# LuoweiZhou/VLP

Measured on NVIDIA H100. Metric: image_text_samples_per_sec, higher is better.
Workload: dtype bf16

## Files before the change

### vlp_b200/csrc/api.cu

```cuda
#include "../../include/vlpk.h"

#include <cstdlib>
#include <cstring>

#include "attn.cuh"
#include "decode.cuh"
#include "gemm.cuh"
#include "head.cuh"
#include "host.cuh"
#include "optim.cuh"
#include "rowops.cuh"
#include "tables.cuh"

using namespace vlpk;
typedef __nv_bfloat16 bf16;

namespace {

inline cudaStream_t S(void* s) { return reinterpret_cast<cudaStream_t>(s); }

enum { SITE_ATTN = 0, SITE_HID1 = 1, SITE_HID2 = 2 };
inline uint64_t site_of(uint64_t layer_id, int site) { return layer_id * 8 + site; }

inline DropoutCfg mk_drop(const VlpkDropout* d, float p, uint64_t site) {
// ... 322 lines not shown
  const long long i = (static_cast<long long>(blockIdx.x) * blockDim.x + threadIdx.x) * 8;
  if (i >= M * N) return;
  const long long r = i / N;
  const int c = static_cast<int>(i % N);
  const uint4 ud = *reinterpret_cast<const uint4*>(dy + r * lddy + c), uy = *reinterpret_cast<const uint4*>(y + r * ldy + c);
  const uint32_t wd[4] = {ud.x, ud.y, ud.z, ud.w}, wy[4] = {uy.x, uy.y, uy.z, uy.w};
  uint32_t o[4];
#pragma unroll
  for (int j = 0; j < 4; ++j) {
    const float2 d = unpack_bf16x2(wd[j]), v = unpack_bf16x2(wy[j]);
    o[j] = pack_bf16x2(v.x > 0.f ? d.x * scale : 0.f, v.y > 0.f ? d.y * scale : 0.f);
  }
  *reinterpret_cast<uint4*>(dpre + i) = make_uint4(o[0], o[1], o[2], o[3]);
}

int score_layer_fwd(const VlpkShape* s, int T, const AttnGroupKv* group, const VlpkLayerWeights* w, const void* x, const uint32_t* key_bits,
                    const uint32_t* query_bits, VlpkLayerActs* a, uint64_t layer_id, cudaStream_t st) {
  const int H = s->H, K = group != nullptr ? T - 1 : s->Lq, R = K + T;
  VLPK_TRY(qkv_fwd(s->B * R, H, w, x, a->qkv, st));
  const bf16* qkv = static_cast<const bf16*>(a->qkv);
  AttnGroupKv g;
  if (group != nullptr) {
    g = *group;
    g.text = qkv + H; g.ld_text = 3 * H; g.T = R; g.pos = 0;
  }
  AttnDesc ad;
  ad.B = s->B; ad.heads = s->heads; ad.Lkv = s->Lkv; ad.kv_slots = s->kv_slots;
  ad.q = qkv; ad.ld_q = 3 * H; ad.q_batch_stride = static_cast<int64_t>(R) * 3 * H;
  ad.k = qkv + H; ad.v = qkv + 2 * H; ad.kv_batch_stride = static_cast<int64_t>(R) * 3 * H;
  ad.ld_kv = group != nullptr ? 2 * H : 3 * H;
  ad.o = a->ctx; ad.ld_o = H; ad.o_batch_stride = static_cast<int64_t>(R) * H;
  ad.lse = a->lse;
  ad.drop = make_dropout(0.f, 0, 0);
  if (K > 0) {
    AttnDesc kd = ad;
    kd.Lq = K;
    kd.mask_bits = key_bits; kd.mask_rows = K;
    VLPK_TRY(launch_attn_fwd(kd, group != nullptr ? &g : nullptr, nullptr, st));
  }
  AttnDesc qd = ad;
  qd.Lq = T;
  qd.q = qkv + static_cast<size_t>(K) * 3 * H;
  qd.o = static_cast<bf16*>(a->ctx) + static_cast<size_t>(K) * H;
  qd.mask_bits = query_bits; qd.mask_rows = T;
  qd.lse = a->lse + static_cast<size_t>(s->B) * s->heads * K;
  AttnSelfKv sk;
  sk.k = qkv + static_cast<size_t>(K) * 3 * H + H;
  sk.v = qkv + static_cast<size_t>(K) * 3 * H + 2 * H;
  sk.ld = 3 * H; sk.batch_stride = static_cast<int64_t>(R) * 3 * H;
  VLPK_TRY(launch_attn_fwd(qd, group != nullptr ? &g : nullptr, &sk, st));
  VlpkShape rows = *s;
  rows.Lq = rows.Lkv = R;
  VLPK_TRY(attn_out_ln(&rows, w, x, a, 0.f, nullptr, layer_id, st));
  return ffn_fwd_impl(&rows, w, a, 0.f, nullptr, layer_id, st);
}

int score_stack_fwd(const VlpkShape* s, int T, int n_layers, const VlpkLayerWeights* w, const void* x, AttnGroupKv* group,
                    const void* const* prefix, const uint32_t* key_bits, const uint32_t* query_bits, VlpkLayerActs* acts, cudaStream_t st) {
  const void* cur = x;
  for (int i = 0; i < n_layers; ++i) {
    if (group != nullptr) group->prefix = prefix[i];
    VLPK_TRY(score_layer_fwd(s, T, group, &w[i], cur, key_bits, query_bits, &acts[i], i, st));
    cur = acts[i].y;
  }
  return 0;
}

size_t act_bytes(const VlpkShape* s, size_t rows, size_t kv_elems) {
  const size_t H = s->H, I = s->I, M = static_cast<size_t>(s->B) * rows;
  const size_t lse = (static_cast<size_t>(s->B) * s->heads * rows + 3) / 4 * 4;
  return 2 * (M * (3 * H + 5 * H + 2 * I) + kv_elems) + 4 * (lse + 4 * M);
}

}

#pragma GCC visibility push(default)
extern "C" {

int vlpk_version(void) { return VLPK_VERSION; }
int vlpk_debug_set_option(const char* name, int value) {
  VLPK_CHECK_ARG(name != nullptr, "set_option: null name");
  if (strcmp(name, "wgrad_stream") == 0) { g_wgrad_stream = value ? 1 : 0; return 0; }
  if (strcmp(name, "attn_tiled") == 0) { set_attn_tiled(value != 0); return 0; }
  set_error("set_option: unknown option '%s'", name);
  return -1;
}
int vlpk_debug_plan_gemm(int M, int N, int K, int a_mn, int b_mn, int nseg, int seg_rows, int epi, int bn, int splits, int* out2) {
  GemmDesc g;
  g.M = M; g.N = N; g.K = K;
  g.a_mn = a_mn != 0; g.b_mn = b_mn != 0;
  g.nseg = nseg; g.b_seg_rows = seg_rows;
  g.epi = epi; g.bn = bn; g.splits = splits;
  return plan_gemm(g, &out2[0], &out2[1]);
}
void vlpk_set_reserved_sms(int n) { set_reserved_sms(n); }
void vlpk_set_deterministic(int on) { set_deterministic(on != 0); }
const char* vlpk_last_error(void) { return get_error(); }

int vlpk_mask_pack(const void* mask, int dtype, int mode, int B, int rows, int kv, int64_t stride_b, int64_t stride_r, uint32_t* out,
                   void* stream) {
  VLPK_CHECK_ARG(mask != nullptr && out != nullptr, "mask_pack: null pointer");
  return launch_mask_pack(mask, dtype, mode, B, rows, kv, stride_b, stride_r, out, S(stream));
}

int vlpk_mask_synth(const int32_t* len_b, const int32_t* mode, int len_a, int B, int L, uint32_t* out, void* stream) {
  return launch_mask_synth(len_b, mode, len_a, B, L, out, S(stream));
}

int vlpk_mask_synth_grouped(const int32_t* len_b, int G, int len_a, int B, int T, uint32_t* out, void* stream) {
  return launch_mask_synth_grouped(len_b, G, len_a, B, T, out, S(stream));
}

int vlpk_linear_fwd(int M, int N, int K, const void* x, int64_t ldx, const void* w, int64_t ldw, const void* bias, void* y, int64_t ldy,
                    int act, const VlpkDropout* drop, uint64_t site, void* stream) {
  VLPK_CHECK_ARG(x && w && y, "linear_fwd: null pointer");
  VLPK_CHECK_ARG(act == VLPK_ACT_NONE || act == VLPK_ACT_RELU, "linear_fwd: act %d unsupported", act);
  const DropoutCfg dc = (act == VLPK_ACT_RELU && drop != nullptr) ? mk_drop(drop, drop->p, site) : make_dropout(0.f, 0, site);
  return fwd_linear(M, N, K, x, ldx, w, ldw, bias, y, ldy, act == VLPK_ACT_RELU ? EPI_RELU : EPI_STORE, nullptr, 0, dc, S(stream));
}

int vlpk_linear_bwd(int M, int N, int K, const void* x, int64_t ldx, const void* w, int64_t ldw, const void* y, int64_t ldy,
                    const void* dy, int64_t lddy, void* dpre, void* dx, int64_t lddx, float* dw, int64_t lddw, float* db, int act,
                    float p_drop, void* stream) {
  VLPK_CHECK_ARG(x && w && dy && dw, "linear_bwd: null pointer");
  cudaStream_t st = S(stream);
  const void* g = dy;
  int64_t ldg = lddy;
  if (act == VLPK_ACT_RELU) {
    VLPK_CHECK_ARG(y != nullptr && dpre != nullptr && N % 8 == 0, "linear_bwd: relu needs y, dpre and N %% 8 == 0");
    const long long n = static_cast<long long>(M) * N;
    LaunchScope scope(CAT_MISC, 6.0 * n, st);
    relu_bwd_kernel<<<static_cast<unsigned>((n / 8 + 255) / 256), 256, 0, st>>>(static_cast<bf16*>(dpre), static_cast<const bf16*>(dy),
                                                                             static_cast<const bf16*>(y), M, N, lddy, ldy,
                                                                             p_drop > 0.f ? 1.0f / (1.0f - p_drop) : 1.0f);
    VLPK_CUDA(cudaGetLastError());
    g = dpre;
    ldg = N;
  }
  if (db != nullptr) VLPK_TRY(launch_colsum(g, ldg, M, N, db, st));
  VLPK_TRY(wgrad_linear(M, N, K, g, ldg, x, ldx, dw, lddw, st));
  if (dx != nullptr) VLPK_TRY(dgrad_linear(M, N, K, g, ldg, w, ldw, dx, lddx, EPI_STORE, nullptr, 0, st));
  return 0;
}

static EmbedArgs mk_embed(int B, int L, int H, int R, int vis_input, const int64_t* ids, const int64_t* tt, const int64_t* pos,
                          const void* word_w, const void* pos_w, const void* type_w, const void* vis, const void* vpe,
                          const void* ln_g) {
  EmbedArgs a;
  a.B = B; a.L = L; a.H = H; a.R = R; a.vis_input = vis_input;
  a.ids = reinterpret_cast<const long long*>(ids);
  a.tt = reinterpret_cast<const long long*>(tt);
  a.pos = reinterpret_cast<const long long*>(pos);
  a.word = static_cast<const bf16*>(word_w); a.posw = static_cast<const bf16*>(pos_w); a.typew = static_cast<const bf16*>(type_w);
  a.vis = static_cast<const bf16*>(vis); a.vpe = static_cast<const bf16*>(vpe);
  a.gamma = static_cast<const bf16*>(ln_g);
  return a;
}

int vlpk_embed_fwd(int B, int L, int H, int R, int vis_input, const int64_t* ids, const int64_t* token_type, const int64_t* pos,
                   const void* word_w, const void* pos_w, const void* type_w, const void* vis, const void* vis_pe, const void* ln_g,
                   const void* ln_b, void* y, float* stats, const VlpkDropout* drop, uint64_t site, void* stream) {
  VLPK_CHECK_ARG(ids && word_w && pos_w && type_w && ln_g && ln_b && y, "embed_fwd: null pointer");
  EmbedArgs a = mk_embed(B, L, H, R, vis_input, ids, token_type, pos, word_w, pos_w, type_w, vis, vis_pe, ln_g);
  a.beta = static_cast<const bf16*>(ln_b);
  a.y = static_cast<bf16*>(y);
  a.stats = reinterpret_cast<float2*>(stats);
// ... 547 lines not shown
```

### vlp_b200/csrc/common.cuh

```cuda
#pragma once
#include <cuda.h>
#include <cuda_bf16.h>
#include <cuda_runtime.h>
#include <stdint.h>

#include "wgmma.cuh"

namespace vlpk {

__device__ __forceinline__ uint32_t smem_u32(const void* p) {
  return static_cast<uint32_t>(__cvta_generic_to_shared(p));
}

__device__ __forceinline__ uint32_t lane_id() { return threadIdx.x & 31u; }

__device__ __forceinline__ bool elect_one() {
  uint32_t pred = 0;
  asm volatile(
      "{\n\t"
      ".reg .pred P;\n\t"
      "elect.sync _|P, 0xffffffff;\n\t"
      "selp.u32 %0, 1, 0, P;\n\t"
      "}\n"
      : "=r"(pred));
  return pred != 0;
}

__device__ __forceinline__ void mbar_init(uint64_t* bar, uint32_t count) {
  asm volatile("mbarrier.init.shared::cta.b64 [%0], %1;" ::"r"(smem_u32(bar)), "r"(count) : "memory");
}
__device__ __forceinline__ void fence_mbar_init() {
  asm volatile("fence.mbarrier_init.release.cluster;" ::: "memory");
}
__device__ __forceinline__ void fence_proxy_async_smem() {
  asm volatile("fence.proxy.async.shared::cta;" ::: "memory");
}
__device__ __forceinline__ void mbar_arrive_expect_tx(uint64_t* bar, uint32_t bytes) {
  asm volatile("mbarrier.arrive.expect_tx.shared::cta.b64 _, [%0], %1;" ::"r"(smem_u32(bar)), "r"(bytes)
               : "memory");
}
__device__ __forceinline__ void mbar_arrive(uint64_t* bar) {
  asm volatile("mbarrier.arrive.shared::cta.b64 _, [%0];" ::"r"(smem_u32(bar)) : "memory");
}
__device__ __forceinline__ bool mbar_try_wait(uint64_t* bar, uint32_t parity) {
  uint32_t ok;
  asm volatile(
      "{\n\t"
      ".reg .pred P;\n\t"
      "mbarrier.try_wait.parity.shared::cta.b64 P, [%1], %2;\n\t"
      "selp.u32 %0, 1, 0, P;\n\t"
      "}\n"
      : "=r"(ok)
      : "r"(smem_u32(bar)), "r"(parity)
      : "memory");
  return ok != 0;
}
__device__ __forceinline__ void mbar_wait(uint64_t* bar, uint32_t parity) {
  uint32_t spins = 0;
  while (!mbar_try_wait(bar, parity)) {
    if (++spins > (1u << 28)) { __trap(); }
  }
}
__device__ __forceinline__ void mbar_wait_flag(uint64_t* bar, uint32_t parity, bool& timed_out) {
  uint32_t spins = 0;
  while (!timed_out && !mbar_try_wait(bar, parity)) {
    if (++spins > (1u << 28)) timed_out = true;
  }
}

__device__ __forceinline__ void pdl_launch_dependents() { asm volatile("griddepcontrol.launch_dependents;" ::: "memory"); }
__device__ __forceinline__ void pdl_wait() { asm volatile("griddepcontrol.wait;" ::: "memory"); }

__device__ __forceinline__ void tma_prefetch_desc(const CUtensorMap* m) {
  asm volatile("prefetch.tensormap [%0];" ::"l"(reinterpret_cast<uint64_t>(m)) : "memory");
}
__device__ __forceinline__ void tma_load_2d(void* dst, const CUtensorMap* m, uint64_t* bar, int c0, int c1) {
  asm volatile(
      "cp.async.bulk.tensor.2d.shared::cluster.global.tile.mbarrier::complete_tx::bytes [%0], [%1, {%3, %4}], [%2];"
      ::"r"(smem_u32(dst)), "l"(reinterpret_cast<uint64_t>(m)), "r"(smem_u32(bar)), "r"(c0), "r"(c1)
      : "memory");
}
__device__ __forceinline__ void tma_load_3d(void* dst, const CUtensorMap* m, uint64_t* bar, int c0, int c1,
                                            int c2) {
  asm volatile(
      "cp.async.bulk.tensor.3d.shared::cluster.global.tile.mbarrier::complete_tx::bytes [%0], [%1, {%3, %4, %5}], "
      "[%2];" ::"r"(smem_u32(dst)),
      "l"(reinterpret_cast<uint64_t>(m)), "r"(smem_u32(bar)), "r"(c0), "r"(c1), "r"(c2)
      : "memory");
}
__device__ __forceinline__ void tma_store_2d(const CUtensorMap* m, const void* src, int c0, int c1) {
  asm volatile("cp.async.bulk.tensor.2d.global.shared::cta.tile.bulk_group [%0, {%2, %3}], [%1];" ::"l"(
                   reinterpret_cast<uint64_t>(m)),
               "r"(smem_u32(src)), "r"(c0), "r"(c1)
               : "memory");
}
__device__ __forceinline__ void tma_store_3d(const CUtensorMap* m, const void* src, int c0, int c1, int c2) {
  asm volatile("cp.async.bulk.tensor.3d.global.shared::cta.tile.bulk_group [%0, {%2, %3, %4}], [%1];" ::"l"(
                   reinterpret_cast<uint64_t>(m)),
               "r"(smem_u32(src)), "r"(c0), "r"(c1), "r"(c2)
               : "memory");
}
__device__ __forceinline__ void tma_reduce_add_2d(const CUtensorMap* m, const void* src, int c0, int c1) {
  asm volatile("cp.reduce.async.bulk.tensor.2d.global.shared::cta.add.tile.bulk_group [%0, {%2, %3}], [%1];" ::"l"(
                   reinterpret_cast<uint64_t>(m)),
               "r"(smem_u32(src)), "r"(c0), "r"(c1)
               : "memory");
}
__device__ __forceinline__ void tma_reduce_add_3d(const CUtensorMap* m, const void* src, int c0, int c1, int c2) {
  asm volatile("cp.reduce.async.bulk.tensor.3d.global.shared::cta.add.tile.bulk_group [%0, {%2, %3, %4}], [%1];" ::"l"(
                   reinterpret_cast<uint64_t>(m)),
               "r"(smem_u32(src)), "r"(c0), "r"(c1), "r"(c2)
               : "memory");
}
__device__ __forceinline__ void tma_store_commit() { asm volatile("cp.async.bulk.commit_group;" ::: "memory"); }
template <int N>
__device__ __forceinline__ void tma_store_wait_read() {
  asm volatile("cp.async.bulk.wait_group.read %0;" ::"n"(N) : "memory");
}
template <int N>
__device__ __forceinline__ void tma_store_wait() {
  asm volatile("cp.async.bulk.wait_group %0;" ::"n"(N) : "memory");
}

__device__ __forceinline__ void wgmma_fence() { asm volatile("wgmma.fence.sync.aligned;" ::: "memory"); }
__device__ __forceinline__ void wgmma_commit() { asm volatile("wgmma.commit_group.sync.aligned;" ::: "memory"); }
template <int N>
__device__ __forceinline__ void wgmma_wait() {
  asm volatile("wgmma.wait_group.sync.aligned %0;" ::"n"(N) : "memory");
}
template <uint32_t N>
__device__ __forceinline__ void setmaxnreg_dec() { asm volatile("setmaxnreg.dec.sync.aligned.u32 %0;" ::"n"(N)); }
template <uint32_t N>
__device__ __forceinline__ void setmaxnreg_inc() { asm volatile("setmaxnreg.inc.sync.aligned.u32 %0;" ::"n"(N)); }
template <int N>
__device__ __forceinline__ void reg_fence(float (&d)[N]) {
#pragma unroll
  for (int i = 0; i < N; ++i) asm volatile("" : "+f"(d[i])::"memory");
}

__device__ __forceinline__ uint64_t wgmma_desc_sw128(uint32_t saddr, uint32_t lbo_bytes, uint32_t sbo_bytes) {
  uint64_t d = 0;
  d |= static_cast<uint64_t>((saddr & 0x3FFFFu) >> 4);
  d |= static_cast<uint64_t>((lbo_bytes >> 4) & 0x3FFFu) << 16;
  d |= static_cast<uint64_t>((sbo_bytes >> 4) & 0x3FFFu) << 32;
  d |= 1ull << 62;
  return d;
}

__device__ __forceinline__ uint32_t pack_bf16x2(float lo, float hi) {
  __nv_bfloat162 v = __floats2bfloat162_rn(lo, hi);
  return *reinterpret_cast<uint32_t*>(&v);
}
__device__ __forceinline__ float2 unpack_bf16x2(uint32_t u) {
  __nv_bfloat162 v = *reinterpret_cast<__nv_bfloat162*>(&u);
  return __bfloat1622float2(v);
}
__device__ __forceinline__ float bf16_round(float x) { return __bfloat162float(__float2bfloat16_rn(x)); }

__device__ __forceinline__ float fast_ex2(float x) {
  float y;
  asm("ex2.approx.ftz.f32 %0, %1;" : "=f"(y) : "f"(x));
  return y;
// ... 81 lines not shown
```

### vlp_b200/csrc/gemm.cu

```cuda
#include "gemm.cuh"

#include <cstdlib>

#include "host.cuh"
#include "rowops.cuh"

namespace vlpk {

static constexpr int BM = 128;
static constexpr int BK = 64;
static constexpr int NUM_THREADS = 384;
static constexpr int PRODUCER_REGS = 24;
static constexpr int CONSUMER_REGS = 240;
static constexpr int STG_BYTES = 64 * 128;
static constexpr int STG_PER_CONSUMER = 4;
static constexpr int SMEM_MAX = 232448;
static constexpr int BN = 128;

struct GemmTmaps {
  CUtensorMap a;
  CUtensorMap b[3];
  CUtensorMap d0;
  CUtensorMap d1;
  CUtensorMap aux;
};

struct GemmArgs {
  int M, N, K;
  int b_seg_rows;
  int splits;
  int split_slices;
  const __nv_bfloat16* bias[3];
  float relu_scale;
  DropoutCfg drop;
  float* colsum;
};

template <int STAGES>
struct SmemLayout {
  static constexpr int A_BYTES = BM * BK * 2;
  static constexpr int B_BYTES = BN * BK * 2;
  static constexpr int STAGE_BYTES = A_BYTES + B_BYTES;
  static constexpr int OFF_STG = STAGES * STAGE_BYTES;
  static constexpr int OFF_BAR = OFF_STG + 2 * STG_PER_CONSUMER * STG_BYTES;
  static constexpr int NUM_BARS = 3 * STAGES + 2;
  static constexpr int TOTAL = OFF_BAR + NUM_BARS * 8;
  static constexpr int DYN_BYTES = TOTAL + 1024;
  static_assert(DYN_BYTES <= SMEM_MAX, "shared memory budget exceeded");
};

struct StageCount {
  static constexpr int value = (SMEM_MAX - 1024 - 2 * STG_PER_CONSUMER * STG_BYTES - 256) / (BM * BK * 2 + BN * BK * 2);
};

__device__ __forceinline__ void wg_bar_sync(int cw) {
  asm volatile("bar.sync %0, 128;" ::"r"(cw + 1) : "memory");
}

template <bool A_MN, bool B_MN, int EPI>
__global__ void __launch_bounds__(NUM_THREADS, 1)
gemm_kernel(const __grid_constant__ GemmTmaps tm, const GemmArgs args) {
  constexpr int STAGES = StageCount::value;
  using L = SmemLayout<STAGES>;
  extern __shared__ uint8_t smem_raw[];
  uint8_t* smem = reinterpret_cast<uint8_t*>((reinterpret_cast<uintptr_t>(smem_raw) + 1023) & ~uintptr_t(1023));

  uint64_t* bars = reinterpret_cast<uint64_t*>(smem + L::OFF_BAR);
  uint64_t* full_bar = bars;
  uint64_t* empty_bar = bars + 2 * STAGES;
  uint64_t* aux_bar = bars + 3 * STAGES;
  constexpr bool HAS_AUX = (EPI == EPI_ADD || EPI == EPI_MUL || EPI == EPI_DRELU);

  pdl_launch_dependents();
  const int wg = __shfl_sync(0xffffffffu, threadIdx.x >> 7, 0);
  const int lane = threadIdx.x & 31;

  const int num_m = (args.M + BM - 1) / BM;
  const int num_n = (args.N + BN - 1) / BN;
  const int total_kb = (args.K + BK - 1) / BK;
  const int kb_per = (total_kb + args.splits - 1) / args.splits;
  const int num_work = num_m * num_n * args.splits;

  if (threadIdx.x == 0) {
    tma_prefetch_desc(&tm.a);
    tma_prefetch_desc(&tm.b[0]);
    tma_prefetch_desc(&tm.d0);
    if (HAS_AUX) tma_prefetch_desc(&tm.aux);
    for (int i = 0; i < 2 * STAGES; ++i) mbar_init(&full_bar[i], 1);
    for (int i = 0; i < STAGES; ++i) mbar_init(&empty_bar[i], 4);
    for (int i = 0; i < 2; ++i) mbar_init(&aux_bar[i], 1);
    fence_mbar_init();
  }
  __syncthreads();
  pdl_wait();

  if (wg == 0) {
    setmaxnreg_dec<PRODUCER_REGS>();
    if (threadIdx.x < 32) {
      int stage = 0;
      uint32_t phase = 0;
      int item = 0;
      for (int w = blockIdx.x; w < num_work; w += gridDim.x, ++item) {
        uint64_t* fb = full_bar + (item & 1) * STAGES;
        const int n_blk = w % num_n;
        const int m_blk = (w / num_n) % num_m;
        const int split = w / (num_n * num_m);
        const int kb0 = split * kb_per;
        const int kb1 = min(total_kb, kb0 + kb_per);
        const int m0 = m_blk * BM;
        for (int kb = kb0; kb < kb1; ++kb) {
          mbar_wait(&empty_bar[stage], phase ^ 1u);
          if (elect_one()) {
            uint8_t* sA = smem + stage * L::STAGE_BYTES;
            uint8_t* sB = sA + L::A_BYTES;
            mbar_arrive_expect_tx(&fb[stage], L::STAGE_BYTES);
            if (!A_MN) {
              tma_load_2d(sA, &tm.a, &fb[stage], kb * BK, m0);
            } else {
#pragma unroll
              for (int j = 0; j < BM / 64; ++j) tma_load_2d(sA + j * 8192, &tm.a, &fb[stage], m0 + j * 64, kb * BK);
            }
            if (!B_MN) {
              const int n0 = n_blk * BN;
              const int seg = n0 / args.b_seg_rows;
              tma_load_2d(sB, &tm.b[seg], &fb[stage], kb * BK, n0 - seg * args.b_seg_rows);
            } else {
              const int k0 = kb * BK;
              const int seg = k0 / args.b_seg_rows;
#pragma unroll
              for (int j = 0; j < BN / 64; ++j)
                tma_load_2d(sB + j * 8192, &tm.b[seg], &fb[stage], n_blk * BN + j * 64, k0 - seg * args.b_seg_rows);
            }
          }
          __syncwarp();
          if (++stage == STAGES) {
            stage = 0;
            phase ^= 1u;
          }
        }
      }
    }
  } else {
    setmaxnreg_inc<CONSUMER_REGS>();
    const int cw = wg - 1;
    const int t = threadIdx.x - 128 * wg;
    const int fr = (t >> 5) * 16 + (lane >> 2);
    const int fc = (lane & 3) * 2;
    const bool store_thread = (t == 0);
    const uint64_t dseed = drop_seed(args.drop);
    constexpr bool HAS_BIAS = !B_MN && (EPI == EPI_STORE || EPI == EPI_GELU || EPI == EPI_RELU);
    uint8_t* stg_base = smem + L::OFF_STG + cw * STG_PER_CONSUMER * STG_BYTES;
    const uint32_t a_base = smem_u32(smem);
    const uint32_t b_base = smem_u32(smem) + L::A_BYTES;
    uint64_t* fb = full_bar + cw * STAGES;
    int stage = 0;
    uint32_t phases = 0;
    uint32_t box_seq = 0;
    uint32_t aux_phase = 0;
    bool timed_out = false;
    float acc[2][BN / 2];
#pragma unroll
    for (int i = 0; i < BN / 2; ++i) acc[0][i] = acc[1][i] = 0.f;
    for (int w = blockIdx.x + cw * gridDim.x; w < num_work; w += 2 * gridDim.x) {
      const int w_other = w - static_cast<int>(gridDim.x);
      if (w_other >= static_cast<int>(blockIdx.x)) {
        const int split_o = w_other / (num_n * num_m);
        const int kb0_o = split_o * kb_per;
        stage = (stage + min(total_kb, kb0_o + kb_per) - kb0_o) % STAGES;
      }
      const int n_blk = w % num_n;
      const int m_blk = (w / num_n) % num_m;
      const int split = w / (num_n * num_m);
      const int kb0 = split * kb_per;
      const int kb1 = min(total_kb, kb0 + kb_per);
      const int n0 = n_blk * BN;

      int prev_stage = 0;
      for (int kb = kb0; kb < kb1; ++kb) {
        mbar_wait_flag(&fb[stage], (phases >> stage) & 1u, timed_out);
        phases ^= 1u << stage;
        const uint32_t sa = a_base + stage * L::STAGE_BYTES;
        const uint32_t sb = b_base + stage * L::STAGE_BYTES;
        reg_fence(acc[0]);
        reg_fence(acc[1]);
        wgmma_fence();
#pragma unroll
        for (int k = 0; k < BK / 16; ++k) {
          const uint64_t bdesc = B_MN ? wgmma_desc_sw128(sb + k * 2048, 8192, 1024) : wgmma_desc_sw128(sb + k * 32, 16, 1024);
#pragma unroll
          for (int h = 0; h < 2; ++h) {
            const uint32_t sah = sa + h * 8192;
            const uint64_t adesc = A_MN ? wgmma_desc_sw128(sah + k * 2048, 8192, 1024) : wgmma_desc_sw128(sah + k * 32, 16, 1024);
            wgmma_m64n128k16_ss<A_MN ? 1 : 0, B_MN ? 1 : 0>(acc[h], adesc, bdesc, (kb > kb0 || k > 0) ? 1u : 0u);
          }
        }
        wgmma_commit();
        if (HAS_AUX && kb == kb0) {
          static_assert(STG_PER_CONSUMER == 2 * (BN / 64), "one staging box per aux box of a tile");
          wg_bar_sync(cw);
          if (store_thread) {
            tma_store_wait_read<0>();
            fence_proxy_async_smem();
            mbar_arrive_expect_tx(&aux_bar[cw], STG_PER_CONSUMER * STG_BYTES);
#pragma unroll
            for (int b = 0; b < STG_PER_CONSUMER; ++b)
              tma_load_2d(stg_base + b * STG_BYTES, &tm.aux, &aux_bar[cw], n0 + (b & 1) * 64, m_blk * BM + (b >> 1) * 64);
          }
        }
        wgmma_wait<1>();
        reg_fence(acc[0]);
        reg_fence(acc[1]);
        if (kb > kb0 && lane == 0) mbar_arrive(&empty_bar[prev_stage]);
        prev_stage = stage;
        if (++stage == STAGES) stage = 0;
      }
      wgmma_wait<0>();
      reg_fence(acc[0]);
      reg_fence(acc[1]);
      if (lane == 0) mbar_arrive(&empty_bar[prev_stage]);

      if (EPI == EPI_REDUCE_F32) {
        constexpr int NBOX = BN / 32;
#pragma unroll
        for (int h = 0; h < 2; ++h) {
          const int m0 = m_blk * BM + h * 64;
#pragma unroll
          for (int c = 0; c < NBOX; ++c) {
            uint8_t* stg = stg_base + (box_seq % STG_PER_CONSUMER) * STG_BYTES;
            if (store_thread) tma_store_wait_read<STG_PER_CONSUMER - 1>();
            wg_bar_sync(cw);
#pragma unroll
            for (int j = 0; j < 8; ++j) {
              const int i = c * 16 + 2 * j;
              const int r = fr + 8 * (j & 1), col = 8 * (j >> 1) + fc;
              *reinterpret_cast<float2*>(stg + r * 128 + (((col >> 2) ^ (r & 7)) << 4) + (col & 3) * 4) = make_float2(acc[h][i], acc[h][i + 1]);
            }
            fence_proxy_async_smem();
            wg_bar_sync(cw);
            if (store_thread) {
              tma_reduce_add_3d(&tm.d0, stg, n0 + c * 32, m0, args.split_slices ? split : 0);
              tma_store_commit();
            }
            ++box_seq;
          }
        }
      } else {
        constexpr int NBOX = BN / 64;
        if (HAS_AUX) {
          mbar_wait_flag(&aux_bar[cw], aux_phase, timed_out);
          aux_phase ^= 1u;
        }
        const __nv_bfloat16* bp = nullptr;
        int bias_off = 0;
        if (HAS_BIAS) {
          const int seg = n0 / args.b_seg_rows;
          bp = args.bias[seg];
          bias_off = seg * args.b_seg_rows;
        }
#pragma unroll
        for (int h = 0; h < 2; ++h) {
          const int m0 = m_blk * BM + h * 64;
          int nh = n0;
          const __nv_bfloat16* bph = bp;
          uint64_t dsh = dseed;
          asm volatile("" : "+r"(nh), "+l"(bph), "+l"(dsh));
#pragma unroll
          for (int c = 0; c < NBOX; ++c) {
            uint8_t* stg = (EPI == EPI_GELU) ? stg_base + (box_seq & 1u) * 2 * STG_BYTES : stg_base + (box_seq % STG_PER_CONSUMER) * STG_BYTES;
            uint8_t* stg_g = stg + STG_BYTES;
            if (store_thread) {
              if (EPI == EPI_GELU) tma_store_wait_read<STG_PER_CONSUMER / 2 - 1>(); else tma_store_wait_read<STG_PER_CONSUMER - 1>();
            }
            wg_bar_sync(cw);
#pragma unroll
            for (int j = 0; j < 16; ++j) {
              const int i = c * 32 + 2 * j;
              const int r = fr + 8 * (j & 1), col = 8 * (j >> 1) + fc;
              const int n = nh + c * 64 + col;
              const long long m = m0 + r;
              const int so = r * 128 + (((col >> 3) ^ (r & 7)) << 4) + (col & 7) * 2;
              float v0 = acc[h][i], v1 = acc[h][i + 1];
              if (HAS_BIAS) {
                if (bph != nullptr && n < args.N) {
                  const float2 bb = unpack_bf16x2(__ldg(reinterpret_cast<const unsigned int*>(bph + n - bias_off)));
                  v0 += bb.x;
                  v1 += bb.y;
                }
              }
              if (EPI == EPI_GELU) {
                float g0, d0, g1, d1;
                gelu_and_grad(v0, g0, d0);
                gelu_and_grad(v1, g1, d1);
                *reinterpret_cast<uint32_t*>(stg + so) = pack_bf16x2(d0, d1);
                *reinterpret_cast<uint32_t*>(stg_g + so) = pack_bf16x2(g0, g1);
                continue;
              }
              if (EPI == EPI_RELU) {
                uint32_t keep = 0xFFu;
                if (args.drop.p > 0.f)
                  keep = dropout_keep8(dsh, args.drop.site, (static_cast<uint64_t>(m) * args.N + (n - fc)) >> 3, args.drop.thresh16);
                v0 = fmaxf(v0, 0.f);
                v1 = fmaxf(v1, 0.f);
                v0 = ((keep >> fc) & 1u) ? v0 * args.drop.scale : 0.f;
                v1 = ((keep >> (fc + 1)) & 1u) ? v1 * args.drop.scale : 0.f;
              } else if (EPI == EPI_ADD || EPI == EPI_MUL || EPI == EPI_DRELU) {
                const float2 x = unpack_bf16x2(*reinterpret_cast<const uint32_t*>(stg + so));
                if (EPI == EPI_ADD) {
                  v0 += x.x;
                  v1 += x.y;
                } else if (EPI == EPI_MUL) {
                  v0 *= x.x;
                  v1 *= x.y;
                } else {
                  v0 = x.x > 0.f ? v0 * args.relu_scale : 0.f;
                  v1 = x.y > 0.f ? v1 * args.relu_scale : 0.f;
                }
              }
              *reinterpret_cast<uint32_t*>(stg + so) = pack_bf16x2(v0, v1);
            }
            fence_proxy_async_smem();
            wg_bar_sync(cw);
            if (store_thread) {
              tma_store_2d(&tm.d0, stg, nh + c * 64, m0);
              if (EPI == EPI_GELU) tma_store_2d(&tm.d1, stg_g, nh + c * 64, m0);
              tma_store_commit();
            }
            if (EPI != EPI_GELU && args.colsum != nullptr) {
              const int col = t & 63, r0 = (t >> 6) * 32;
              float acc_c = 0.f;
#pragma unroll 8
              for (int rr = r0; rr < r0 + 32; ++rr) {
                const __nv_bfloat16 v = *reinterpret_cast<const __nv_bfloat16*>(stg + rr * 128 + (((col >> 3) ^ (rr & 7)) << 4) + (col & 7) * 2);
                acc_c += __bfloat162float(v);
              }
              if (nh + c * 64 + col < args.N) atomicAdd(args.colsum + nh + c * 64 + col, acc_c);
            }
            ++box_seq;
          }
        }
      }
    }
    if (store_thread) tma_store_wait<0>();
    if (timed_out) __trap();
  }
}

template <bool A_MN, bool B_MN, int EPI>
static int launch_inst(const GemmTmaps& tm, const GemmArgs& args, int num_work, cudaStream_t stream) {
  constexpr int STAGES = StageCount::value;
  using L = SmemLayout<STAGES>;
  auto kfn = gemm_kernel<A_MN, B_MN, EPI>;
  static bool attr_set = false;
  if (!attr_set) {
    VLPK_CUDA(cudaFuncSetAttribute(kfn, cudaFuncAttributeMaxDynamicSharedMemorySize, L::DYN_BYTES));
    attr_set = true;
  }
  const int max_ctas = gemm_sms();
  const int ctas = num_work < max_ctas ? num_work : max_ctas;
  LaunchScope scope(A_MN ? CAT_GEMM_WGRAD : (B_MN ? CAT_GEMM_DGRAD : CAT_GEMM_FWD), 2.0 * args.M * args.N * args.K, stream);
  VLPK_CUDA(launch_ex(kfn, dim3(ctas), dim3(NUM_THREADS), L::DYN_BYTES, stream, 1, tm, args));
  return 0;
}

static int dispatch(const GemmDesc& g, const GemmTmaps& tm, const GemmArgs& args, int num_work, cudaStream_t s) {
  if (!g.a_mn && !g.b_mn) {
    switch (g.epi) {
      case EPI_STORE: return launch_inst<false, false, EPI_STORE>(tm, args, num_work, s);
      case EPI_GELU: return launch_inst<false, false, EPI_GELU>(tm, args, num_work, s);
      case EPI_RELU: return launch_inst<false, false, EPI_RELU>(tm, args, num_work, s);
      default: break;
    }
  } else if (!g.a_mn && g.b_mn) {
    switch (g.epi) {
      case EPI_STORE: return launch_inst<false, true, EPI_STORE>(tm, args, num_work, s);
      case EPI_ADD: return launch_inst<false, true, EPI_ADD>(tm, args, num_work, s);
      case EPI_MUL: return launch_inst<false, true, EPI_MUL>(tm, args, num_work, s);
      case EPI_DRELU: return launch_inst<false, true, EPI_DRELU>(tm, args, num_work, s);
      case EPI_REDUCE_F32: return launch_inst<false, true, EPI_REDUCE_F32>(tm, args, num_work, s);
      default: break;
    }
  } else if (g.a_mn && g.b_mn) {
    if (g.epi == EPI_REDUCE_F32) return launch_inst<true, true, EPI_REDUCE_F32>(tm, args, num_work, s);
    if (g.epi == EPI_STORE) return launch_inst<true, true, EPI_STORE>(tm, args, num_work, s);
  }
  set_error("gemm: unsupported (a_mn=%d, b_mn=%d, epi=%d) combination", (int)g.a_mn, (int)g.b_mn, g.epi);
  return -1;
}

static double tile_cost(int M, int N, int total_kb, int splits, bool reduce) {
  const int num_m = (M + BM - 1) / BM;
  const int num_n = (N + BN - 1) / BN;
  const long long tiles = static_cast<long long>(num_m) * num_n * splits;
  const int slots = deterministic() ? num_sms() : gemm_sms();
  const long long rounds = (tiles + slots - 1) / slots;
  const int kb_per = (total_kb + splits - 1) / splits;
  const double mainloop = kb_per * (128.0 + double(BN));
  const double epi = (reduce ? 3.0 : 1.5) * BN;
  return rounds * (mainloop + epi + 60.0);
}

int plan_gemm(const GemmDesc& g, int* bn_out, int* splits_out) {
  const int seg_rows = g.nseg > 1 ? g.b_seg_rows : (g.b_mn ? g.K : g.N);
  const int total_kb = (g.K + BK - 1) / BK;
  const bool reduce = (g.epi == EPI_REDUCE_F32);
  VLPK_CHECK_ARG(g.bn == 0 || g.bn == BN, "gemm: no valid tile configuration (bn=%d; tiles are %d wide)", g.bn, BN);
  VLPK_CHECK_ARG(g.nseg == 1 || seg_rows % (g.b_mn ? BK : BN) == 0, "gemm: segment rows %d not tile aligned", seg_rows);
  int splits = 1;
  if (reduce) {
    const int max_s = total_kb / 8 > 0 ? total_kb / 8 : 1;
    if (g.splits > 0) {
      splits = g.splits < max_s ? g.splits : max_s;
    } else {
      double best = 1e300;
      for (int s = 1; s <= max_s; ++s) {
        const double c = tile_cost(g.M, g.N, total_kb, s, reduce);
        if (c < best) {
          best = c;
          splits = s;
        }
      }
    }
  }
  if (splits > total_kb) splits = total_kb;
  {
    const int kb_per = (total_kb + splits - 1) / splits;
    splits = (total_kb + kb_per - 1) / kb_per;
  }
  *bn_out = BN;
  *splits_out = splits;
  return 0;
}

int launch_gemm(const GemmDesc& g, cudaStream_t stream) {
  VLPK_CHECK_ARG(g.M > 0 && g.N > 0 && g.K > 0, "gemm: empty problem M=%d N=%d K=%d", g.M, g.N, g.K);
  VLPK_CHECK_ARG(g.N % 8 == 0, "gemm: N=%d must be a multiple of 8", g.N);
  VLPK_CHECK_ARG(g.nseg >= 1 && g.nseg <= 3, "gemm: nseg=%d", g.nseg);
  const int seg_rows = g.nseg > 1 ? g.b_seg_rows : (g.b_mn ? g.K : g.N);
  const bool reduce = (g.epi == EPI_REDUCE_F32);
  VLPK_CHECK_ARG(g.splits <= 1 || reduce, "gemm: split-K needs EPI_REDUCE_F32");
  VLPK_CHECK_ARG(g.b_rows == 0 || (g.nseg == 1 && g.b_rows <= (g.b_mn ? g.K : g.N)), "gemm: b_rows=%d needs a single B segment", g.b_rows);

  int bn = BN, splits = 1;
  VLPK_TRY(plan_gemm(g, &bn, &splits));

  GemmTmaps tm;
  memset(&tm, 0, sizeof(tm));
  if (!g.a_mn) {
    VLPK_TRY(make_tmap_2d(&tm.a, TM_BF16, g.A, g.K, g.M, g.lda, BK, BM));
  } else {
    VLPK_TRY(make_tmap_2d(&tm.a, TM_BF16, g.A, g.M, g.K, g.lda, 64, BK));
  }
  for (int s = 0; s < g.nseg; ++s) {
    if (!g.b_mn) {
      const int rows = g.nseg > 1 ? seg_rows : (g.b_rows > 0 ? g.b_rows : g.N);
      VLPK_TRY(make_tmap_2d(&tm.b[s], TM_BF16, g.B[s], g.K, rows, g.ldb, BK, bn));
    } else {
      const int rows = g.nseg > 1 ? seg_rows : (g.b_rows > 0 ? g.b_rows : g.K);
      VLPK_TRY(make_tmap_2d(&tm.b[s], TM_BF16, g.B[s], g.N, rows, g.ldb, 64, BK));
    }
  }
  for (int s = g.nseg; s < 3; ++s) tm.b[s] = tm.b[0];
  if (reduce) {
    VLPK_CHECK_ARG(g.split_stride == 0 || (g.split_stride % 4 == 0 && g.split_stride >= static_cast<int64_t>(g.M) * g.ldd0),
                   "gemm: split_stride %lld must be a multiple of 4 and cover M x ldd0", (long long)g.split_stride);
    const uint64_t dims[3] = {static_cast<uint64_t>(g.N), static_cast<uint64_t>(g.M), static_cast<uint64_t>(g.split_stride ? splits : 1)};
    const uint64_t strides[2] = {static_cast<uint64_t>(g.ldd0) * 4,
                                 static_cast<uint64_t>(g.split_stride ? g.split_stride : static_cast<int64_t>(g.M) * g.ldd0) * 4};
    const uint32_t box[3] = {32, 64, 1};
    VLPK_TRY(make_tmap(&tm.d0, TM_F32, 3, g.D0, dims, strides, box));
    tm.d1 = tm.d0;
  } else {
    VLPK_TRY(make_tmap_2d(&tm.d0, TM_BF16, g.D0, g.N, g.M, g.ldd0, 64, 64));
    if (g.epi == EPI_GELU) {
      VLPK_CHECK_ARG(g.D1 != nullptr, "gemm: EPI_GELU needs D1");
      VLPK_TRY(make_tmap_2d(&tm.d1, TM_BF16, g.D1, g.N, g.M, g.ldd1, 64, 64));
    } else {
      tm.d1 = tm.d0;
    }
  }
  VLPK_CHECK_ARG(g.colsum == nullptr || (!reduce && g.epi != EPI_GELU), "gemm: colsum fusion is for single-output bf16 epilogues");
  if (g.epi == EPI_ADD || g.epi == EPI_MUL || g.epi == EPI_DRELU) {
    VLPK_CHECK_ARG(g.aux != nullptr && (g.ld_aux % 8) == 0 && (reinterpret_cast<uintptr_t>(g.aux) & 15u) == 0,
                   "gemm: aux must be 16-byte aligned with ld %% 8 == 0");
    VLPK_TRY(make_tmap_2d(&tm.aux, TM_BF16, g.aux, g.N, g.M, g.ld_aux, 64, 64));
  } else {
    tm.aux = tm.d0;
  }

  GemmArgs a;
  a.M = g.M;
  a.N = g.N;
  a.K = g.K;
  a.b_seg_rows = seg_rows;
  a.splits = splits;
  a.split_slices = (reduce && g.split_stride > 0) ? 1 : 0;
  for (int s = 0; s < 3; ++s) a.bias[s] = (s < g.nseg) ? g.bias[s] : nullptr;
  a.relu_scale = g.relu_scale;
  a.colsum = g.colsum;
  a.drop = g.drop;

  const int num_m = (g.M + BM - 1) / BM;
  const int num_n = (g.N + bn - 1) / bn;
  const int num_work = num_m * num_n * splits;
  return dispatch(g, tm, a, num_work, stream);
}

int launch_gemm_split_slices(GemmDesc g, int slot, cudaStream_t stream) {
  VLPK_CHECK_ARG(g.epi == EPI_REDUCE_F32 && g.split_stride == 0, "gemm: split slices are for EPI_REDUCE_F32 into one D0");
  int bn = 0, splits = 1;
  VLPK_TRY(plan_gemm(g, &bn, &splits));
  if (splits == 1) return launch_gemm(g, stream);
  VLPK_CHECK_ARG(g.ldd0 == g.N, "gemm: split slices need a dense D0 (ldd0 %lld != N %d)", (long long)g.ldd0, g.N);
  const long long n = static_cast<long long>(g.M) * g.N;
  float* part = scratch_f32(slot, static_cast<size_t>(n) * splits, stream);
  if (part == nullptr) return -1;
  VLPK_CUDA(cudaMemsetAsync(part, 0, static_cast<size_t>(n) * splits * sizeof(float), stream));
  float* out = static_cast<float*>(g.D0);
  g.D0 = part;
  g.splits = splits;
  g.split_stride = n;
  VLPK_TRY(launch_gemm(g, stream));
  return launch_sum_parts(part, splits, n, out, stream);
}

}
```

### vlp_b200/csrc/gemm.cuh

```cuda
#pragma once
#include "common.cuh"

namespace vlpk {

enum Epi : int {
  EPI_STORE = 0,
  EPI_GELU = 1,
  EPI_RELU = 2,
  EPI_ADD = 3,
  EPI_MUL = 4,
  EPI_DRELU = 5,
  EPI_REDUCE_F32 = 6,
};

struct GemmDesc {
  int M = 0, N = 0, K = 0;
  bool a_mn = false;
  const void* A = nullptr;
  int64_t lda = 0;
  bool b_mn = false;
  int nseg = 1;
  const void* B[3] = {nullptr, nullptr, nullptr};
  int64_t ldb = 0;
  int b_seg_rows = 0;
  int b_rows = 0;
  const __nv_bfloat16* bias[3] = {nullptr, nullptr, nullptr};
  void* D0 = nullptr;
  int64_t ldd0 = 0;
  void* D1 = nullptr;
  int64_t ldd1 = 0;
  const __nv_bfloat16* aux = nullptr;
  int64_t ld_aux = 0;
  int epi = EPI_STORE;
  float relu_scale = 1.0f;
  DropoutCfg drop = {0.f, 1.f, 0u, 0ull, 0ull, nullptr};
  float* colsum = nullptr;
  int splits = 1;
  int64_t split_stride = 0;
  int bn = 0;
};

int launch_gemm(const GemmDesc& g, cudaStream_t stream);
int plan_gemm(const GemmDesc& g, int* bn_out, int* splits_out);
int launch_gemm_split_slices(GemmDesc g, int slot, cudaStream_t stream);

}
```

Baseline: 5342.

## Multicast B tiles across 2-CTA clusters in the persistent GEMM kernel

Launches the persistent warp-specialized GEMM as 2-CTA clusters along M. Each CTA loads one 64-column half of the shared B tile and multicasts it via TMA to both CTAs, which halves B global/L2 traffic. Empty barriers now count arrivals from both CTAs, and cluster syncs are added at start and end. The cost is cross-CTA coupling that can stall a pair, odd-M padding waste, and occupancy limited by the cluster count.

```diff
diff --git a/vlp_b200/csrc/api.cu b/vlp_b200/csrc/api.cu
--- a/vlp_b200/csrc/api.cu
+++ b/vlp_b200/csrc/api.cu
@@ -428,6 +428,7 @@
   VLPK_CHECK_ARG(name != nullptr, "set_option: null name");
   if (strcmp(name, "wgrad_stream") == 0) { g_wgrad_stream = value ? 1 : 0; return 0; }
   if (strcmp(name, "attn_tiled") == 0) { set_attn_tiled(value != 0); return 0; }
+  if (strcmp(name, "gemm_cluster") == 0) { set_gemm_cluster(value != 0); return 0; }
   set_error("set_option: unknown option '%s'", name);
   return -1;
 }
diff --git a/vlp_b200/csrc/common.cuh b/vlp_b200/csrc/common.cuh
--- a/vlp_b200/csrc/common.cuh
+++ b/vlp_b200/csrc/common.cuh
@@ -42,6 +42,15 @@
 __device__ __forceinline__ void mbar_arrive(uint64_t* bar) {
   asm volatile("mbarrier.arrive.shared::cta.b64 _, [%0];" ::"r"(smem_u32(bar)) : "memory");
 }
+__device__ __forceinline__ void mbar_arrive_cluster(uint64_t* bar, uint32_t cta) {
+  asm volatile(
+      "{\n\t"
+      ".reg .b32 ra;\n\t"
+      "mapa.shared::cluster.u32 ra, %0, %1;\n\t"
+      "mbarrier.arrive.release.cluster.shared::cluster.b64 _, [ra];\n\t"
+      "}\n" ::"r"(smem_u32(bar)), "r"(cta)
+      : "memory");
+}
 __device__ __forceinline__ bool mbar_try_wait(uint64_t* bar, uint32_t parity) {
   uint32_t ok;
   asm volatile(
@@ -71,6 +80,15 @@
 __device__ __forceinline__ void pdl_launch_dependents() { asm volatile("griddepcontrol.launch_dependents;" ::: "memory"); }
 __device__ __forceinline__ void pdl_wait() { asm volatile("griddepcontrol.wait;" ::: "memory"); }
 
+__device__ __forceinline__ uint32_t cluster_ctarank() {
+  uint32_t r;
+  asm volatile("mov.u32 %0, %%cluster_ctarank;" : "=r"(r));
+  return r;
+}
+__device__ __forceinline__ void cluster_sync() {
+  asm volatile("barrier.cluster.arrive.release;\n\tbarrier.cluster.wait.acquire;" ::: "memory");
+}
+
 __device__ __forceinline__ void tma_prefetch_desc(const CUtensorMap* m) {
   asm volatile("prefetch.tensormap [%0];" ::"l"(reinterpret_cast<uint64_t>(m)) : "memory");
 }
@@ -78,6 +96,13 @@
   asm volatile(
       "cp.async.bulk.tensor.2d.shared::cluster.global.tile.mbarrier::complete_tx::bytes [%0], [%1, {%3, %4}], [%2];"
       ::"r"(smem_u32(dst)), "l"(reinterpret_cast<uint64_t>(m)), "r"(smem_u32(bar)), "r"(c0), "r"(c1)
+      : "memory");
+}
+__device__ __forceinline__ void tma_load_2d_multicast(void* dst, const CUtensorMap* m, uint64_t* bar, int c0, int c1, uint16_t cta_mask) {
+  asm volatile(
+      "cp.async.bulk.tensor.2d.shared::cluster.global.tile.mbarrier::complete_tx::bytes.multicast::cluster [%0], [%1, {%3, %4}], [%2], "
+      "%5;" ::"r"(smem_u32(dst)),
+      "l"(reinterpret_cast<uint64_t>(m)), "r"(smem_u32(bar)), "r"(c0), "r"(c1), "h"(cta_mask)
       : "memory");
 }
 __device__ __forceinline__ void tma_load_3d(void* dst, const CUtensorMap* m, uint64_t* bar, int c0, int c1,
diff --git a/vlp_b200/csrc/gemm.cu b/vlp_b200/csrc/gemm.cu
--- a/vlp_b200/csrc/gemm.cu
+++ b/vlp_b200/csrc/gemm.cu
@@ -30,6 +30,8 @@
   int b_seg_rows;
   int splits;
   int split_slices;
+  int cluster;
+  int num_mp;
   const __nv_bfloat16* bias[3];
   float relu_scale;
   DropoutCfg drop;
@@ -53,6 +55,8 @@
   static constexpr int value = (SMEM_MAX - 1024 - 2 * STG_PER_CONSUMER * STG_BYTES - 256) / (BM * BK * 2 + BN * BK * 2);
 };
 
+__device__ __forceinline__ int cluster_rank(int csize) { return csize > 1 ? static_cast<int>(cluster_ctarank()) : 0; }
+
 __device__ __forceinline__ void wg_bar_sync(int cw) {
   asm volatile("bar.sync %0, 128;" ::"r"(cw + 1) : "memory");
 }
@@ -75,11 +79,14 @@
   const int wg = __shfl_sync(0xffffffffu, threadIdx.x >> 7, 0);
   const int lane = threadIdx.x & 31;
 
-  const int num_m = (args.M + BM - 1) / BM;
+  const int csize = args.cluster;
+  const int cid = blockIdx.x >> (csize - 1);
+  const int num_clusters = gridDim.x >> (csize - 1);
+  const int num_mp = args.num_mp;
   const int num_n = (args.N + BN - 1) / BN;
   const int total_kb = (args.K + BK - 1) / BK;
   const int kb_per = (total_kb + args.splits - 1) / args.splits;
-  const int num_work = num_m * num_n * args.splits;
+  const int num_work = num_mp * num_n * args.splits;
 
   if (threadIdx.x == 0) {
     tma_prefetch_desc(&tm.a);
@@ -87,11 +94,11 @@
     tma_prefetch_desc(&tm.d0);
     if (HAS_AUX) tma_prefetch_desc(&tm.aux);
     for (int i = 0; i < 2 * STAGES; ++i) mbar_init(&full_bar[i], 1);
-    for (int i = 0; i < STAGES; ++i) mbar_init(&empty_bar[i], 4);
+    for (int i = 0; i < STAGES; ++i) mbar_init(&empty_bar[i], 4 * csize);
     for (int i = 0; i < 2; ++i) mbar_init(&aux_bar[i], 1);
     fence_mbar_init();
   }
-  __syncthreads();
+  if (csize > 1) cluster_sync(); else __syncthreads();
   pdl_wait();
 
   if (wg == 0) {
@@ -100,11 +107,11 @@
       int stage = 0;
       uint32_t phase = 0;
       int item = 0;
-      for (int w = blockIdx.x; w < num_work; w += gridDim.x, ++item) {
+      for (int w = cid; w < num_work; w += num_clusters, ++item) {
         uint64_t* fb = full_bar + (item & 1) * STAGES;
         const int n_blk = w % num_n;
-        const int m_blk = (w / num_n) % num_m;
-        const int split = w / (num_n * num_m);
+        const int m_blk = (w / num_n) % num_mp * csize + cluster_rank(csize);
+        const int split = w / (num_n * num_mp);
         const int kb0 = split * kb_per;
         const int kb1 = min(total_kb, kb0 + kb_per);
         const int m0 = m_blk * BM;
@@ -120,16 +127,23 @@
 #pragma unroll
               for (int j = 0; j < BM / 64; ++j) tma_load_2d(sA + j * 8192, &tm.a, &fb[stage], m0 + j * 64, kb * BK);
             }
-            if (!B_MN) {
-              const int n0 = n_blk * BN;
-              const int seg = n0 / args.b_seg_rows;
-              tma_load_2d(sB, &tm.b[seg], &fb[stage], kb * BK, n0 - seg * args.b_seg_rows);
-            } else {
-              const int k0 = kb * BK;
-              const int seg = k0 / args.b_seg_rows;
-#pragma unroll
-              for (int j = 0; j < BN / 64; ++j)
-                tma_load_2d(sB + j * 8192, &tm.b[seg], &fb[stage], n_blk * BN + j * 64, k0 - seg * args.b_seg_rows);
+            const int j0 = csize > 1 ? cluster_ctarank() : 0;
+            const int j1 = csize > 1 ? j0 + 1 : BN / 64;
+            for (int j = j0; j < j1; ++j) {
+              int c0, c1, seg;
+              if (!B_MN) {
+                const int n0 = n_blk * BN;
+                seg = n0 / args.b_seg_rows;
+                c0 = kb * BK;
+                c1 = n0 - seg * args.b_seg_rows + j * 64;
+              } else {
+                const int k0 = kb * BK;
+                seg = k0 / args.b_seg_rows;
+                c0 = n_blk * BN + j * 64;
+                c1 = k0 - seg * args.b_seg_rows;
+              }
+              if (csize > 1) tma_load_2d_multicast(sB + j * 8192, &tm.b[seg], &fb[stage], c0, c1, 0x3);
+              else tma_load_2d(sB + j * 8192, &tm.b[seg], &fb[stage], c0, c1);
             }
           }
           __syncwarp();
@@ -161,16 +175,20 @@
     float acc[2][BN / 2];
 #pragma unroll
     for (int i = 0; i < BN / 2; ++i) acc[0][i] = acc[1][i] = 0.f;
-    for (int w = blockIdx.x + cw * gridDim.x; w < num_work; w += 2 * gridDim.x) {
-      const int w_other = w - static_cast<int>(gridDim.x);
-      if (w_other >= static_cast<int>(blockIdx.x)) {
-        const int split_o = w_other / (num_n * num_m);
+    auto release = [&](int s) {
+      mbar_arrive(&empty_bar[s]);
+      if (csize > 1) mbar_arrive_cluster(&empty_bar[s], cluster_ctarank() ^ 1u);
+    };
+    for (int w = cid + cw * num_clusters; w < num_work; w += 2 * num_clusters) {
+      const int w_other = w - num_clusters;
+      if (w_other >= cid) {
+        const int split_o = w_other / (num_n * num_mp);
         const int kb0_o = split_o * kb_per;
         stage = (stage + min(total_kb, kb0_o + kb_per) - kb0_o) % STAGES;
       }
       const int n_blk = w % num_n;
-      const int m_blk = (w / num_n) % num_m;
-      const int split = w / (num_n * num_m);
+      const int m_blk = (w / num_n) % num_mp * csize + cluster_rank(csize);
+      const int split = w / (num_n * num_mp);
       const int kb0 = split * kb_per;
       const int kb1 = min(total_kb, kb0 + kb_per);
       const int n0 = n_blk * BN;
@@ -210,14 +228,14 @@
         wgmma_wait<1>();
         reg_fence(acc[0]);
         reg_fence(acc[1]);
-        if (kb > kb0 && lane == 0) mbar_arrive(&empty_bar[prev_stage]);
+        if (kb > kb0 && lane == 0) release(prev_stage);
         prev_stage = stage;
         if (++stage == STAGES) stage = 0;
       }
       wgmma_wait<0>();
       reg_fence(acc[0]);
       reg_fence(acc[1]);
-      if (lane == 0) mbar_arrive(&empty_bar[prev_stage]);
+      if (lane == 0) release(prev_stage);
 
       if (EPI == EPI_REDUCE_F32) {
         constexpr int NBOX = BN / 32;
@@ -343,45 +361,68 @@
     if (store_thread) tma_store_wait<0>();
     if (timed_out) __trap();
   }
-}
+  if (csize > 1) cluster_sync();
+}
+
+static bool g_gemm_cluster = true;
+void set_gemm_cluster(bool on) { g_gemm_cluster = on; }
 
 template <bool A_MN, bool B_MN, int EPI>
-static int launch_inst(const GemmTmaps& tm, const GemmArgs& args, int num_work, cudaStream_t stream) {
+static int launch_inst(const GemmTmaps& tm, GemmArgs args, int num_m, int num_n, cudaStream_t stream) {
   constexpr int STAGES = StageCount::value;
   using L = SmemLayout<STAGES>;
   auto kfn = gemm_kernel<A_MN, B_MN, EPI>;
-  static bool attr_set = false;
-  if (!attr_set) {
+  static int max_clusters = -1;
+  if (max_clusters < 0) {
     VLPK_CUDA(cudaFuncSetAttribute(kfn, cudaFuncAttributeMaxDynamicSharedMemorySize, L::DYN_BYTES));
-    attr_set = true;
-  }
-  const int max_ctas = gemm_sms();
-  const int ctas = num_work < max_ctas ? num_work : max_ctas;
+    cudaLaunchConfig_t cfg;
+    memset(&cfg, 0, sizeof(cfg));
+    cfg.gridDim = dim3(2);
+    cfg.blockDim = dim3(NUM_THREADS);
+    cfg.dynamicSmemBytes = L::DYN_BYTES;
+    cudaLaunchAttribute attr;
+    attr.id = cudaLaunchAttributeClusterDimension;
+    attr.val.clusterDim.x = 2;
+    attr.val.clusterDim.y = 1;
+    attr.val.clusterDim.z = 1;
+    cfg.attrs = &attr;
+    cfg.numAttrs = 1;
+    int n = 0;
+    VLPK_CUDA(cudaOccupancyMaxActiveClusters(&n, kfn, &cfg));
+    max_clusters = n;
+  }
+  const int sms = gemm_sms();
+  args.cluster = (g_gemm_cluster && sms >= 2 && max_clusters >= 1) ? 2 : 1;
+  args.num_mp = (num_m + args.cluster - 1) / args.cluster;
+  const long long work = static_cast<long long>(args.num_mp) * num_n * args.splits;
+  long long slots = sms / args.cluster;
+  if (args.cluster > 1 && slots > max_clusters) slots = max_clusters;
+  const int ctas = static_cast<int>((work < slots ? work : slots) * args.cluster);
   LaunchScope scope(A_MN ? CAT_GEMM_WGRAD : (B_MN ? CAT_GEMM_DGRAD : CAT_GEMM_FWD), 2.0 * args.M * args.N * args.K, stream);
-  VLPK_CUDA(launch_ex(kfn, dim3(ctas), dim3(NUM_THREADS), L::DYN_BYTES, stream, 1, tm, args));
+  VLPK_CUDA(launch_ex(kfn, dim3(ctas), dim3(NUM_THREADS), L::DYN_BYTES, stream, args.cluster, tm, args));
   return 0;
 }
 
-static int dispatch(const GemmDesc& g, const GemmTmaps& tm, const GemmArgs& args, int num_work, cudaStream_t s) {
+static int dispatch(const GemmDesc& g, const GemmTmaps& tm, const GemmArgs& args, int num_m, int num_n, cudaStream_t s) {
   if (!g.a_mn && !g.b_mn) {
     switch (g.epi) {
-      case EPI_STORE: return launch_inst<false, false, EPI_STORE>(tm, args, num_work, s);
-      case EPI_GELU: return launch_inst<false, false, EPI_GELU>(tm, args, num_work, s);
-      case EPI_RELU: return launch_inst<false, false, EPI_RELU>(tm, args, num_work, s);
+      case EPI_STORE: return launch_inst<false, false, EPI_STORE>(tm, args, num_m, num_n, s);
+      case EPI_GELU: return launch_inst<false, false, EPI_GELU>(tm, args, num_m, num_n, s);
+      case EPI_RELU: return launch_inst<false, false, EPI_RELU>(tm, args, num_m, num_n, s);
       default: break;
     }
   } else if (!g.a_mn && g.b_mn) {
     switch (g.epi) {
-      case EPI_STORE: return launch_inst<false, true, EPI_STORE>(tm, args, num_work, s);
-      case EPI_ADD: return launch_inst<false, true, EPI_ADD>(tm, args, num_work, s);
-      case EPI_MUL: return launch_inst<false, true, EPI_MUL>(tm, args, num_work, s);
-      case EPI_DRELU: return launch_inst<false, true, EPI_DRELU>(tm, args, num_work, s);
-      case EPI_REDUCE_F32: return launch_inst<false, true, EPI_REDUCE_F32>(tm, args, num_work, s);
+      case EPI_STORE: return launch_inst<false, true, EPI_STORE>(tm, args, num_m, num_n, s);
+      case EPI_ADD: return launch_inst<false, true, EPI_ADD>(tm, args, num_m, num_n, s);
+      case EPI_MUL: return launch_inst<false, true, EPI_MUL>(tm, args, num_m, num_n, s);
+      case EPI_DRELU: return launch_inst<false, true, EPI_DRELU>(tm, args, num_m, num_n, s);
+      case EPI_REDUCE_F32: return launch_inst<false, true, EPI_REDUCE_F32>(tm, args, num_m, num_n, s);
       default: break;
     }
   } else if (g.a_mn && g.b_mn) {
-    if (g.epi == EPI_REDUCE_F32) return launch_inst<true, true, EPI_REDUCE_F32>(tm, args, num_work, s);
-    if (g.epi == EPI_STORE) return launch_inst<true, true, EPI_STORE>(tm, args, num_work, s);
+    if (g.epi == EPI_REDUCE_F32) return launch_inst<true, true, EPI_REDUCE_F32>(tm, args, num_m, num_n, s);
+    if (g.epi == EPI_STORE) return launch_inst<true, true, EPI_STORE>(tm, args, num_m, num_n, s);
   }
   set_error("gemm: unsupported (a_mn=%d, b_mn=%d, epi=%d) combination", (int)g.a_mn, (int)g.b_mn, g.epi);
   return -1;
@@ -453,7 +494,7 @@
   for (int s = 0; s < g.nseg; ++s) {
     if (!g.b_mn) {
       const int rows = g.nseg > 1 ? seg_rows : (g.b_rows > 0 ? g.b_rows : g.N);
-      VLPK_TRY(make_tmap_2d(&tm.b[s], TM_BF16, g.B[s], g.K, rows, g.ldb, BK, bn));
+      VLPK_TRY(make_tmap_2d(&tm.b[s], TM_BF16, g.B[s], g.K, rows, g.ldb, BK, 64));
     } else {
       const int rows = g.nseg > 1 ? seg_rows : (g.b_rows > 0 ? g.b_rows : g.K);
       VLPK_TRY(make_tmap_2d(&tm.b[s], TM_BF16, g.B[s], g.N, rows, g.ldb, 64, BK));
@@ -499,10 +540,9 @@
   a.colsum = g.colsum;
   a.drop = g.drop;
 
-  const int num_m = (g.M + BM - 1) / BM;
-  const int num_n = (g.N + bn - 1) / bn;
-  const int num_work = num_m * num_n * splits;
-  return dispatch(g, tm, a, num_work, stream);
+  a.cluster = 1;
+  a.num_mp = 0;
+  return dispatch(g, tm, a, (g.M + BM - 1) / BM, (g.N + bn - 1) / bn, stream);
 }
 
 int launch_gemm_split_slices(GemmDesc g, int slot, cudaStream_t stream) {
diff --git a/vlp_b200/csrc/gemm.cuh b/vlp_b200/csrc/gemm.cuh
--- a/vlp_b200/csrc/gemm.cuh
+++ b/vlp_b200/csrc/gemm.cuh
@@ -43,5 +43,6 @@
 int launch_gemm(const GemmDesc& g, cudaStream_t stream);
 int plan_gemm(const GemmDesc& g, int* bn_out, int* splits_out);
 int launch_gemm_split_slices(GemmDesc g, int slot, cudaStream_t stream);
+void set_gemm_cluster(bool on);
 
 }
```

Result: slower. 3335, median of 6 (-37.6%).
